# LahiruCooray/rl-aerial-manipulator

Hardware: NVIDIA B200
Metric: env_steps_per_sec (higher is better)
Workload: dtype f32

## Files before the change

### rl-aerial-manipulator_b200/csrc/qs_rollout_impl.cuh

```cuda
#include "../../include/quadsim.h"
#include "qs_internal.cuh"
#include "qs_tc.cuh"

#include <stdio.h>

#if !defined(QS_RO_NS) || !defined(QS_RO_EPI_SPLIT) || !defined(QS_RO_ENV_SPLIT) || !(defined(QS_RO_BUILD_FUSED) || defined(QS_RO_BUILD_POLICY))
#error "include qs_rollout_impl.cuh from qs_rollout.cu / qs_rollout_policy.cu"
#endif

namespace qs {
namespace QS_RO_NS {
using namespace tc;

constexpr int EPI_SPLIT = QS_RO_EPI_SPLIT, ENV_SPLIT = QS_RO_ENV_SPLIT;
constexpr int HEAD_SPLIT = EPI_SPLIT < 2 ? EPI_SPLIT : 2;
__host__ __device__ constexpr int chunk_owner(int ch) { return EPI_SPLIT == 3 ? (ch < 4 ? ch % 3 : (ch - 3) % 3) : ch % EPI_SPLIT; }
constexpr int EPI_WARPS = 8 * EPI_SPLIT, ENV_WARPS = 4 * ENV_SPLIT, MMA_WARPS = 2;
#ifndef QS_RO_ENV_FIRST
#define QS_RO_ENV_FIRST 0
#endif
#ifndef QS_RO_LDBUF
#define QS_RO_LDBUF 1
#endif
#ifndef QS_RO_LD_SPLIT
#define QS_RO_LD_SPLIT 0
#endif
#ifndef QS_RO_ST16
#ifdef QS_RO_BUILD_POLICY
#define QS_RO_ST16 1
#else
#define QS_RO_ST16 0
#endif
#endif
constexpr int W_EPI0 = QS_RO_ENV_FIRST ? ENV_WARPS : 0, W_ENV0 = QS_RO_ENV_FIRST ? 0 : EPI_WARPS, W_MMA0 = EPI_WARPS + ENV_WARPS;
constexpr int RO_WARPS = ((EPI_WARPS + ENV_WARPS + MMA_WARPS + 3) / 4) * 4;
constexpr int RO_THREADS = RO_WARPS * 32;
constexpr int REGS_LAUNCH = (65536 / RO_THREADS) / 8 * 8;
#ifdef QS_RO_BUILD_FUSED
constexpr bool REBALANCE = REGS_LAUNCH < 128;
#else
constexpr bool REBALANCE = false;
#endif
constexpr int REGS_MMA = 40;
constexpr int REGS_ENV = EPI_SPLIT == 1 ? 128 : 152;
constexpr int REGS_EPI = EPI_SPLIT == 1 ? 88 : 72;
static_assert(!REBALANCE || (EPI_WARPS * REGS_EPI + ENV_WARPS * REGS_ENV + 4 * REGS_MMA) * 32 <= RO_THREADS * REGS_LAUNCH, "register pool of the CTA");
static_assert(!REBALANCE || (EPI_WARPS % 4 == 0 && ENV_WARPS % 4 == 0), "setmaxnreg works on whole warpgroups");
constexpr int XBUFS = ENV_SPLIT == 2 ? 2 : 3;

constexpr uint32_t SLOT_COLS = 256, C_D1 = 0, C_D2 = 128, C_D3 = 192;

constexpr int IMG_WHI = 0, IMG_WLO = W_SET, IMG_CONST = 2 * W_SET;
constexpr int IMG_BYTES = IMG_CONST + ((C_TOTAL * 4 + 127) / 128) * 128;
constexpr int X_HALF = (K1 / 8) * ROWS * 16;
constexpr int X_BYTES = 2 * X_HALF;
constexpr int ONE_BYTES = 2 * ROWS * 16;
constexpr int X_LBO = ROWS * 16;
constexpr int SM_ONE = IMG_BYTES;
constexpr int SM_X = SM_ONE + ONE_BYTES;
constexpr int SM_OUT_MEAN = SM_X + XBUFS * X_BYTES;
constexpr int SM_OUT_VAL = SM_OUT_MEAN + 2 * HEAD_SPLIT * ROWS * 16;
constexpr int SM_TILE = SM_OUT_VAL + 2 * HEAD_SPLIT * ROWS * 4;
constexpr int SM_MOM = SM_TILE + ENV_WARPS * 32 * 21 * 4;
constexpr int SM_NORM = SM_MOM + ENV_WARPS * 40 * 8;
constexpr int SM_BARS = SM_NORM + 3 * 32 * 4;
enum : int { B_XFULL = 0 , B_XFREE = 3 , B_D1 = 6, B_D2 = 8, B_D3 = 10, B_H1 = 12, B_H2 = 20, B_D3FREE = 24, B_OUTF = 26, B_OUTE = 34, N_BARS = 42 };
constexpr int SM_MISC = SM_BARS + N_BARS * 8;
constexpr int SM_TOTAL = SM_MISC + 16;
static_assert(SM_TOTAL <= 232448, "shared memory budget of one CTA on B200");
static_assert(SM_X % 128 == 0 && SM_ONE % 128 == 0, "operand tiles are 128-byte aligned");

__device__ int g_ro_status;

#ifdef QS_RO_TRACE
constexpr int TRACE_LEN = 2048;
__device__ uint2 g_ro_trace[32][TRACE_LEN];
#define RO_TRACE_INIT() uint2* tr_buf = g_ro_trace[threadIdx.x >> 5]; int tr_n = 0; const bool tr_on = blockIdx.x == 0 && (threadIdx.x & 31) == 0
#define RO_TRACE(code) do { if (tr_on && tr_n < TRACE_LEN - 1) tr_buf[tr_n++] = make_uint2((uint32_t)(code), (uint32_t)clock64()); } while (0)
#define RO_TRACE_END() do { if (tr_on) tr_buf[TRACE_LEN - 1] = make_uint2((uint32_t)tr_n, 0u); } while (0)
#else
#define RO_TRACE_INIT() do { } while (0)
#define RO_TRACE(code) do { } while (0)
#define RO_TRACE_END() do { } while (0)
#endif

struct RoParams {
    const unsigned char* image;
    const float* params;
    const float* obs;
    const double* norm;
    float norm_eps, norm_clip;
    int sample_mode;
    const float* noise;
    uint64_t noise_seed;
    unsigned long long* noise_step;
    float lo[4], hi[4];
    float* obs_norm_out;
    float* actions;
    float* actions_clipped;
    float* values;
    float* logp;
    int64_t n;
    StepParams<float> sp;
    double* mom_out;
    double* mom_merge;
    unsigned int* ticket;
};

__device__ __forceinline__ void mbar_arrive(uint32_t bar) {
    asm volatile("mbarrier.arrive.shared::cta.b64 _, [%0];" ::"r"(bar) : "memory");
}
#ifndef QS_RO_WAIT_HINT_NS
#define QS_RO_WAIT_HINT_NS 20000
#endif
#ifndef QS_RO_BACKOFF_NS
#define QS_RO_BACKOFF_NS 0
#endif
__device__ __forceinline__ uint32_t mbar_try(uint32_t bar, uint32_t parity) {
    uint32_t ok;
#if QS_RO_WAIT_HINT_NS > 0
    asm volatile(
        "{\n\t"
        ".reg .pred p;\n\t"
        "mbarrier.try_wait.parity.shared::cta.b64 p, [%1], %2, %3;\n\t"
        "selp.u32 %0, 1, 0, p;\n\t"
        "}\n"
        : "=r"(ok)
        : "r"(bar), "r"(parity), "r"((uint32_t)QS_RO_WAIT_HINT_NS)
        : "memory");
#else
    asm volatile(
        "{\n\t"
        ".reg .pred p;\n\t"
        "mbarrier.try_wait.parity.shared::cta.b64 p, [%1], %2;\n\t"
        "selp.u32 %0, 1, 0, p;\n\t"
        "}\n"
        : "=r"(ok)
        : "r"(bar), "r"(parity)
        : "memory");
#endif
    return ok;
}
__device__ __forceinline__ uint32_t mbar_test(uint32_t bar, uint32_t parity) {
    uint32_t ok;
    asm volatile(
        "{\n\t"
        ".reg .pred p;\n\t"
        "mbarrier.test_wait.parity.shared::cta.b64 p, [%1], %2;\n\t"
        "selp.u32 %0, 1, 0, p;\n\t"
        "}\n"
        : "=r"(ok)
        : "r"(bar), "r"(parity)
        : "memory");
    return ok;
}
#ifndef QS_RO_TIGHT_WAIT
#define QS_RO_TIGHT_WAIT 1
#endif
__device__ __forceinline__ bool mbar_wait_slow(uint32_t bar, uint32_t parity, int code) {
#if QS_RO_TIGHT_WAIT
    uint32_t ok;
    asm volatile(
        "{\n\t"
        ".reg .pred p, q;\n\t"
        ".reg .u32 n;\n\t"
        "mov.u32 n, 0;\n\t"
        "QS_WAIT_LOOP:\n\t"
        "mbarrier.try_wait.parity.shared::cta.b64 p, [%1], %2, %3;\n\t"
        "@p bra QS_WAIT_DONE;\n\t"
        "add.u32 n, n, 1;\n\t"
        "setp.lt.u32 q, n, 4194304;\n\t"
        "@q bra QS_WAIT_LOOP;\n\t"
        "QS_WAIT_DONE:\n\t"
        "selp.u32 %0, 1, 0, p;\n\t"
        "}\n"
        : "=r"(ok)
        : "r"(bar), "r"(parity), "r"((uint32_t)(QS_RO_WAIT_HINT_NS > 0 ? QS_RO_WAIT_HINT_NS : 1000))
        : "memory");
    if (ok) return true;
#else
    for (uint32_t it = 0; it < (1u << 17); ++it) {
#if QS_RO_BACKOFF_NS > 0
        __nanosleep(QS_RO_BACKOFF_NS);
#endif
        if (mbar_try(bar, parity)) return true;
        if ((it & 0xFF) == 0xFF && *reinterpret_cast<volatile int*>(&g_ro_status) != 0) break;
    }
#endif
    atomicCAS(&g_ro_status, 0, code);
    return false;
}
__device__ __forceinline__ bool mbar_wait_bounded(uint32_t bar, uint32_t parity, int code) {
    if (mbar_try(bar, parity)) return true;
    return mbar_wait_slow(bar, parity, code);
}
#ifndef QS_RO_LAZY_WAIT_NS
#define QS_RO_LAZY_WAIT_NS 600
#endif
__device__ __forceinline__ bool mbar_wait_lazy(uint32_t bar, uint32_t parity, int code) {
#if QS_RO_LAZY_WAIT_NS > 0
    if (mbar_test(bar, parity)) return true;
    for (uint32_t it = 0; it < (1u << 22); ++it) {
        __nanosleep(QS_RO_LAZY_WAIT_NS);
        if (mbar_test(bar, parity)) return true;
    }
    atomicCAS(&g_ro_status, 0, code);
    return false;
#else
    return mbar_wait_bounded(bar, parity, code);
#endif
}
__device__ __forceinline__ void umma_ss(uint32_t tmem_d, uint64_t adesc, uint64_t bdesc, uint32_t idesc, uint32_t accumulate) {
    asm volatile(
        "{\n\t"
        ".reg .pred p;\n\t"
        "setp.ne.b32 p, %4, 0;\n\t"
        "tcgen05.mma.cta_group::1.kind::f16 [%0], %1, %2, %3, p;\n\t"
        "}\n" ::"r"(tmem_d), "l"(adesc), "l"(bdesc), "r"(idesc), "r"(accumulate)
        : "memory");
}
__device__ __forceinline__ void split_h2_rn(float a, float b, uint32_t& hi, uint32_t& lo) {
    asm("cvt.rn.f16x2.f32 %0, %1, %2;" : "=r"(hi) : "f"(b), "f"(a));
#ifdef QS_X_NOSPLIT
    lo = hi ^ 0x3C003C00u;
    return;
#endif
#ifdef QS_X_TRUNCSPLIT
    split_h2(a, b, hi, lo);
    return;
#endif
    float la, lb;
    asm("{\n\t"
        ".reg .f16 l, h, m;\n\t"
        "mov.b32 {l, h}, %2;\n\t"
        "mov.b16 m, 0xBC00;\n\t"
        "fma.rn.f32.f16 %0, l, m, %3;\n\t"
        "fma.rn.f32.f16 %1, h, m, %4;\n\t"
        "}\n"
        : "=f"(la), "=f"(lb)
        : "r"(hi), "f"(a), "f"(b));
    asm("cvt.rn.f16x2.f32 %0, %1, %2;" : "=r"(lo) : "f"(lb), "f"(la));
}
__device__ __forceinline__ void put32_rn(uint32_t taddr, const float* y) {
    uint32_t h[16], l[16];
#pragma unroll
    for (int j = 0; j < 16; ++j) split_h2_rn(y[2 * j], y[2 * j + 1], h[j], l[j]);
    tmem_st16(taddr, h);
    tmem_st16(taddr + 16, l);
}

struct Ctx {
    uint32_t sbase;
    uint32_t tmem;
    int cnt;
    __device__ __forceinline__ uint32_t bar(int idx) const { return sbase + SM_BARS + 8u * (uint32_t)idx; }
};

__device__ __forceinline__ void issue_l1(const Ctx& c, uint32_t d1, int xb, int net) {
    const uint32_t idesc = make_idesc(N1);
    const uint32_t xa = c.sbase + SM_X + xb * X_BYTES;
    const uint32_t wh = c.sbase + IMG_WHI + OFF_W1 + net * W1_BYTES, wl = c.sbase + IMG_WLO + OFF_W1 + net * W1_BYTES;
    constexpr uint32_t B_LBO = N1 * 16;
#pragma unroll
    for (int ks = 0; ks < K1 / 16; ++ks) {
        const uint64_t ah = make_desc(xa + ks * 2 * X_LBO, X_LBO, 128), al = make_desc(xa + X_HALF + ks * 2 * X_LBO, X_LBO, 128);
        const uint64_t bh = make_desc(wh + ks * 2 * B_LBO, B_LBO, 128), bl = make_desc(wl + ks * 2 * B_LBO, B_LBO, 128);
        umma_ss(d1, ah, bh, idesc, ks ? 1u : 0u);
        umma_ss(d1, ah, bl, idesc, 1);
        umma_ss(d1, al, bh, idesc, 1);
    }
}
__device__ __forceinline__ void issue_bias(const Ctx& c, uint32_t d, uint32_t wh, uint32_t wl, int bias_ks) {
    constexpr uint32_t B_LBO = N2 * 16;
    const uint32_t idesc = make_idesc(N2);
    const uint64_t one = make_desc(c.sbase + SM_ONE, X_LBO, 128);
    umma_ss(d, one, make_desc(wh + bias_ks * 2 * B_LBO, B_LBO, 128), idesc, 0);
    umma_ss(d, one, make_desc(wl + bias_ks * 2 * B_LBO, B_LBO, 128), idesc, 1);
}
__device__ __forceinline__ void issue_chunk(uint32_t d, uint32_t a_col, int ch, uint32_t wh, uint32_t wl) {
    constexpr uint32_t B_LBO = N2 * 16;
    const uint32_t idesc = make_idesc(N2);
#pragma unroll
    for (int j = 0; j < 2; ++j) {
        const int ks = 2 * ch + j;
        const uint32_t a_hi = a_col + 32u * ch + (QS_RO_LD_SPLIT ? 16u : 8u) * j;
        const uint64_t bh = make_desc(wh + ks * 2 * B_LBO, B_LBO, 128), bl = make_desc(wl + ks * 2 * B_LBO, B_LBO, 128);
        umma_ts(d, a_hi, bh, idesc, 1);
        umma_ts(d, a_hi, bl, idesc, 1);
        umma_ts(d, a_hi + (QS_RO_LD_SPLIT ? 8u : 16u), bh, idesc, 1);
    }
}

__device__ __forceinline__ void role_mma(const Ctx& c, int slot) {
    const uint32_t d1 = c.tmem + slot * SLOT_COLS + C_D1, d2 = c.tmem + slot * SLOT_COLS + C_D2, d3 = c.tmem + slot * SLOT_COLS + C_D3;
    const int role = 300 + slot * 50;
    uint32_t job = 0;
    bool l1_issued = false;
    RO_TRACE_INIT();
    for (int i = slot; i < c.cnt; i += 2) {
        const int xb = i % XBUFS;
#pragma unroll 1
        for (int net = 0; net < 2; ++net, ++job) {
            const uint32_t par = job & 1u;
            const uint32_t w2h = c.sbase + IMG_WHI + OFF_W2 + net * W2_BYTES, w2l = c.sbase + IMG_WLO + OFF_W2 + net * W2_BYTES;
            const uint32_t w3h = c.sbase + IMG_WHI + OFF_W3 + net * W3_BYTES, w3l = c.sbase + IMG_WLO + OFF_W3 + net * W3_BYTES;
            if (!l1_issued) {
                if (net == 0 && !mbar_wait_bounded(c.bar(B_XFULL + xb), (uint32_t)(i / XBUFS) & 1u, role + B_XFULL + 1)) return;
                tc_fence_after();
                if (elect_one()) {
                    issue_l1(c, d1, xb, net);
                    umma_commit(c.bar(B_D1 + slot));
                    if (net == 1) umma_commit(c.bar(B_XFREE + xb));
                }
                __syncwarp();
                RO_TRACE(0x200000u | job);
            }
            l1_issued = false;
            if (elect_one()) issue_bias(c, d2, w2h, w2l, N1 / 16);
            __syncwarp();
#pragma unroll 1
            for (int ch = 0; ch < 4; ++ch) {
                if (!mbar_wait_bounded(c.bar(B_H1 + slot * 4 + ch), par, role + B_H1 + 1)) return;
                RO_TRACE(0x210000u | (ch << 12) | job);
                tc_fence_after();
                if (elect_one()) {
                    issue_chunk(d2, d1, ch, w2h, w2l);
                    if (ch == 3) umma_commit(c.bar(B_D2 + slot));
                }
                __syncwarp();
            }
            RO_TRACE(0x220000u | job);
            int nxb = xb, nnet = 1, ni = i;
            bool have_next = true;
            if (net == 1) { ni = i + 2; nnet = 0; nxb = ni % XBUFS; have_next = ni < c.cnt; }
            bool l1_now = have_next && (net == 0 || mbar_test(c.bar(B_XFULL + nxb), (uint32_t)(ni / XBUFS) & 1u));
            l1_now = __shfl_sync(0xffffffffu, l1_now ? 1 : 0, 0) != 0;
            if (l1_now) {
                tc_fence_after();
                if (elect_one()) {
                    issue_l1(c, d1, nxb, nnet);
                    umma_commit(c.bar(B_D1 + slot));
                    if (nnet == 1) umma_commit(c.bar(B_XFREE + nxb));
                }
                __syncwarp();
                l1_issued = true;
                RO_TRACE(0x230000u | job);
            }
            if (!mbar_wait_bounded(c.bar(B_D3FREE + slot), par ^ 1u, role + B_D3FREE + 1)) return;
            RO_TRACE(0x240000u | job);
            tc_fence_after();
            if (elect_one()) issue_bias(c, d3, w3h, w3l, N2 / 16);
            __syncwarp();
#pragma unroll 1
            for (int ch = 0; ch < 2; ++ch) {
                if (!mbar_wait_bounded(c.bar(B_H2 + slot * 2 + ch), par, role + B_H2 + 1)) return;
                RO_TRACE(0x250000u | (ch << 12) | job);
                tc_fence_after();
                if (elect_one()) {
                    issue_chunk(d3, d2, ch, w3h, w3l);
                    if (ch == 1) umma_commit(c.bar(B_D3 + slot));
                }
                __syncwarp();
            }
            RO_TRACE(0x260000u | job);
        }
    }
    RO_TRACE_END();
}

__device__ __forceinline__ void tmem_st4(uint32_t taddr, const uint32_t* v) {
    asm volatile("tcgen05.st.sync.aligned.32x32b.x4.b32 [%0], {%1, %2, %3, %4};\n" ::"r"(taddr), "r"(v[0]), "r"(v[1]), "r"(v[2]), "r"(v[3]) : "memory");
}
__device__ __forceinline__ void tmem_ld16(uint32_t taddr, uint32_t* v) {
    asm volatile(
        "tcgen05.ld.sync.aligned.32x32b.x16.b32 {%0, %1, %2, %3, %4, %5, %6, %7, %8, %9, %10, %11, %12, %13, %14, %15}, [%16];\n"
        : "=r"(v[0]), "=r"(v[1]), "=r"(v[2]), "=r"(v[3]), "=r"(v[4]), "=r"(v[5]), "=r"(v[6]), "=r"(v[7]), "=r"(v[8]), "=r"(v[9]),
          "=r"(v[10]), "=r"(v[11]), "=r"(v[12]), "=r"(v[13]), "=r"(v[14]), "=r"(v[15])
        : "r"(taddr));
}
__device__ __forceinline__ void tmem_ld_wait16(uint32_t* v) {
    asm volatile("tcgen05.wait::ld.sync.aligned;"
                 : "+r"(v[0]), "+r"(v[1]), "+r"(v[2]), "+r"(v[3]), "+r"(v[4]), "+r"(v[5]), "+r"(v[6]), "+r"(v[7]), "+r"(v[8]), "+r"(v[9]),
                   "+r"(v[10]), "+r"(v[11]), "+r"(v[12]), "+r"(v[13]), "+r"(v[14]), "+r"(v[15])
                 :
                 : "memory");
}
__device__ __forceinline__ void tanh_split8(const uint32_t* v, uint32_t hi_col, uint32_t lo_col) {
    float y[8];
    tanh8_from_exponents(v, y);
    uint32_t h[4], l[4];
#pragma unroll
    for (int j = 0; j < 4; ++j) split_h2_rn(y[2 * j], y[2 * j + 1], h[j], l[j]);
    tmem_st4(hi_col, h);
    tmem_st4(lo_col, l);
}
__device__ __forceinline__ void chunk_tanh_split(uint32_t col) {
    uint32_t v[32];
#if QS_RO_LD_SPLIT
    tmem_ld16(col, v);
    tmem_ld_wait16(v);
    tmem_ld16(col + 16u, v + 16);
    tanh_split8(v, col, col + 8u);
    tanh_split8(v + 8, col + 4u, col + 12u);
    tmem_ld_wait16(v + 16);
    tanh_split8(v + 16, col + 16u, col + 24u);
    tanh_split8(v + 24, col + 20u, col + 28u);
#else
    tmem_ld32(col, v);
    tmem_ld_wait32(v);
#if QS_RO_ST16
    uint32_t h[16], l[16];
#pragma unroll
    for (int sb = 0; sb < 4; ++sb) {
        float y[8];
        tanh8_from_exponents(v + 8 * sb, y);
#pragma unroll
        for (int j = 0; j < 4; ++j) split_h2_rn(y[2 * j], y[2 * j + 1], h[4 * sb + j], l[4 * sb + j]);
    }
    asm volatile(
        "{\n\t"
        ".reg .b32 a2;\n\t"
        "add.u32 a2, %0, 16;\n\t"
        "tcgen05.st.sync.aligned.32x32b.x16.b32 [%0], {%1, %2, %3, %4, %5, %6, %7, %8, %9, %10, %11, %12, %13, %14, %15, %16};\n\t"
        "tcgen05.st.sync.aligned.32x32b.x16.b32 [a2], {%17, %18, %19, %20, %21, %22, %23, %24, %25, %26, %27, %28, %29, %30, %31, %32};\n\t"
        "}\n" ::"r"(col),
        "r"(h[0]), "r"(h[1]), "r"(h[2]), "r"(h[3]), "r"(h[4]), "r"(h[5]), "r"(h[6]), "r"(h[7]), "r"(h[8]), "r"(h[9]), "r"(h[10]), "r"(h[11]), "r"(h[12]),
        "r"(h[13]), "r"(h[14]), "r"(h[15]), "r"(l[0]), "r"(l[1]), "r"(l[2]), "r"(l[3]), "r"(l[4]), "r"(l[5]), "r"(l[6]), "r"(l[7]), "r"(l[8]), "r"(l[9]),
        "r"(l[10]), "r"(l[11]), "r"(l[12]), "r"(l[13]), "r"(l[14]), "r"(l[15])
        : "memory");
#else
#pragma unroll
    for (int sb = 0; sb < 4; ++sb) tanh_split8(v + 8 * sb, col + 4u * sb, col + 16u + 4u * sb);
#endif
#endif
}

#ifndef QS_RO_DEFER_HEAD
#define QS_RO_DEFER_HEAD 1
#endif
#ifndef QS_RO_HEAD_SCALAR_VF
#ifdef QS_RO_BUILD_POLICY
#define QS_RO_HEAD_SCALAR_VF 1
#else
#define QS_RO_HEAD_SCALAR_VF 0
#endif
#endif
__device__ __forceinline__ void role_epilogue(const Ctx& c, int slot, int half, int quad, int lane, const float* sC, float4* s_mean, float* s_val) {
    const uint32_t tm = c.tmem + slot * SLOT_COLS + ((uint32_t)(quad * 32) << 16);
    const int role = 100 + slot * 50;
    const int row = quad * 32 + lane;
    const uint32_t njobs = c.cnt > slot ? 2u * (uint32_t)((c.cnt - slot + 1) / 2) : 0u;
    float mean[NACT] = {0.f, 0.f, 0.f, 0.f};
    RO_TRACE_INIT();
#pragma unroll 1
    for (uint32_t job = 0; job < njobs + QS_RO_DEFER_HEAD; ++job) {
        const uint32_t par = job & 1u;
        const bool live = job < njobs;
#pragma unroll 1
        for (int stage = 0; stage < 3; ++stage) {
            if (stage == (QS_RO_DEFER_HEAD ? 1 : 2)) {
                if (QS_RO_DEFER_HEAD ? job == 0 : !live) continue;
                if (half >= HEAD_SPLIT) continue;
                const uint32_t hj = job - QS_RO_DEFER_HEAD, hpar = hj & 1u;
                const int net = (int)(hj & 1u);
                const uint32_t k = hj >> 1;
                if (!mbar_wait_bounded(c.bar(B_D3 + slot), hpar, role + B_D3 + 1)) return;
                RO_TRACE(0x130000u | hj);
                tc_fence_after();
                float o[NACT];
#pragma unroll
                for (int j = 0; j < NACT; ++j) o[j] = half == 0 ? sC[C_BH + net * NACT + j] : 0.f;
#pragma unroll 1
                for (int ch = half; ch < 2; ch += HEAD_SPLIT) {
                    uint32_t v[32];
                    tmem_ld32(tm + C_D3 + 32u * (uint32_t)ch, v);
                    tmem_ld_wait32(v);
                    if (ch + HEAD_SPLIT >= 2) {
                        tc_fence_before();
                        __syncwarp();
                        if (lane == 0) mbar_arrive(c.bar(B_D3FREE + slot));
                    }
                    const float4* wh = reinterpret_cast<const float4*>(sC + C_WH + net * N3 * NACT) + 32 * ch;
#pragma unroll
                    for (int sb = 0; sb < 4; ++sb) {
                        float y[8];
                        tanh8_from_exponents(v + 8 * sb, y);
#if QS_RO_HEAD_SCALAR_VF
                        if (net == 1) {
                            const float* w1 = reinterpret_cast<const float*>(wh + 8 * sb);
#pragma unroll
                            for (int q = 0; q < 8; ++q) o[0] = fmaf(y[q], w1[4 * q], o[0]);
                        } else
#endif
                        {
#pragma unroll
                            for (int q = 0; q < 8; ++q) {
                                const float4 w = wh[8 * sb + q];
                                o[0] = fmaf(y[q], w.x, o[0]); o[1] = fmaf(y[q], w.y, o[1]); o[2] = fmaf(y[q], w.z, o[2]); o[3] = fmaf(y[q], w.w, o[3]);
                            }
                        }
                    }
                }
                RO_TRACE(0x140000u | hj);
                if (net == 0) {
#pragma unroll
                    for (int j = 0; j < NACT; ++j) mean[j] = o[j];
                } else {
                    if (!mbar_wait_bounded(c.bar(B_OUTE + slot * 4 + quad), (k & 1u) ^ 1u, role + B_OUTE + 1)) return;
                    s_mean[(slot * HEAD_SPLIT + half) * ROWS + row] = make_float4(mean[0], mean[1], mean[2], mean[3]);
                    s_val[(slot * HEAD_SPLIT + half) * ROWS + row] = o[0];
                    __syncwarp();
                    if (lane == 0) mbar_arrive(c.bar(B_OUTF + slot * 4 + quad));
                }
            } else {
                if (!live) continue;
                const bool first = stage == 0;
                if (EPI_SPLIT == 3 && !first && half == 0) continue;
                if (!mbar_wait_bounded(c.bar((first ? B_D1 : B_D2) + slot), par, role + (first ? B_D1 : B_D2) + 1)) return;
                tc_fence_after();
#pragma unroll 1
                for (int ch = (first ? 0 : 4); ch < (first ? 4 : 6); ++ch) {
                    if (chunk_owner(ch) != half) continue;
                    RO_TRACE(0x100000u | (ch << 12) | job);
                    chunk_tanh_split(tm + 32u * (uint32_t)ch);
                    tmem_st_wait();
                    tc_fence_before();
                    __syncwarp();
                    if (lane == 0) mbar_arrive(c.bar(first ? B_H1 + slot * 4 + ch : B_H2 + slot * 2 + (ch - 4)));
                    RO_TRACE(0x110000u | (ch << 12) | job);
                }
            }
        }
    }
    RO_TRACE_END();
}

__device__ __forceinline__ float4 philox_normal4(uint64_t seed, uint64_t gid, unsigned long long step) {
    uint32_t w[4];
    philox4x32_10((uint32_t)gid, (uint32_t)(gid >> 32), (uint32_t)step, (uint32_t)(step >> 32), (uint32_t)seed ^ 0x85A308D3u,
                  (uint32_t)(seed >> 32) ^ 0x243F6A88u, w);
    float z[4];
#pragma unroll
    for (int j = 0; j < 2; ++j) {
        const float u1 = ((float)(w[2 * j] >> 9) + 0.5f) * 1.1920928955078125e-07f;
        const float th = (float)(w[2 * j + 1] >> 8) * 3.7450702829239286e-07f;
        const float r = sqrtf(-1.3862943611198906f * __log2f(u1));
        float s, co;
        __sincosf(th, &s, &co);
        z[2 * j] = r * co;
        z[2 * j + 1] = r * s;
    }
    return make_float4(z[0], z[1], z[2], z[3]);
}

template <int OBS>
__device__ __forceinline__ bool stage_x(const Ctx& c, const RoParams& p, int i, int quad, int lane, unsigned char* smem, const float* s_norm) {
    const int xb = i % XBUFS;
    if (!mbar_wait_bounded(c.bar(B_XFREE + xb), ((uint32_t)(i / XBUFS) & 1u) ^ 1u, 200 + B_XFREE + 1)) return false;
    const int row = quad * 32 + lane;
    const int64_t tile = (int64_t)blockIdx.x + (int64_t)i * gridDim.x;
    const int64_t e = tile * ROWS + row;
    float x[K1];
#pragma unroll
    for (int k = 0; k < K1; ++k) x[k] = 0.f;
    if (e < p.n) {
        const float* src = p.obs + e * OBS;
        if (OBS % 4 == 0) {
#pragma unroll
            for (int k = 0; k < OBS / 4; ++k) {
                const float4 q = __ldcs(reinterpret_cast<const float4*>(src) + k);
                x[4 * k] = q.x; x[4 * k + 1] = q.y; x[4 * k + 2] = q.z; x[4 * k + 3] = q.w;
            }
        } else {
#pragma unroll
            for (int k = 0; k < OBS; ++k) x[k] = __ldcs(src + k);
        }
        const int64_t e_pf = e + (int64_t)3 * gridDim.x * ROWS;
        if (e_pf < p.n) {
            const char* nr = reinterpret_cast<const char*>(p.obs + e_pf * OBS);
            asm volatile("prefetch.global.L2 [%0];" ::"l"(nr));
            asm volatile("prefetch.global.L2 [%0];" ::"l"(nr + OBS * 4 - 4));
// ... 154 lines not shown
            const int rows = rem < 32 ? (rem < 0 ? 0 : (int)rem) : 32;
            if (rows > 0) warp_store_rows<OBS>(sp.obs_out + e0 * OBS, tile_s, lane, rows);
            if (moments && lane < OBS && rows > 0) {
                const float L = tile_s[lane];
                double t1 = 0.0, t2 = 0.0;
#pragma unroll
                for (int r0 = 0; r0 < 32; r0 += 8) {
                    float a1 = 0.f, a2 = 0.f;
#pragma unroll
                    for (int r = r0; r < r0 + 8; ++r) {
                        const float v = r < rows ? tile_s[r * (OBS + 1) + lane] - L : 0.f;
                        a1 += v;
                        a2 = fmaf(v, v, a2);
                    }
                    t1 += (double)a1;
                    t2 += (double)a2;
                }
                const double dl = (double)L - G;
                m1 += t1 + (double)rows * dl;
                m2 += t2 + 2.0 * dl * t1 + (double)rows * dl * dl;
            }
            __syncwarp();
        }
    }
    if (moments && lane < OBS) { s_mom[lane] = m1; s_mom[OBS + lane] = m2; }
    RO_TRACE_END();
}

template <int VER, bool FUSED>
__global__ void __launch_bounds__(RO_THREADS, 1) rollout_kernel(const RoParams p) {
    constexpr int OBS = EnvTraits<VER>::OBS;
    extern __shared__ __align__(128) unsigned char smem[];
    const int tid = threadIdx.x, warp = tid >> 5, lane = tid & 31;
    float* sC = reinterpret_cast<float*>(smem + IMG_CONST);
    float4* s_mean = reinterpret_cast<float4*>(smem + SM_OUT_MEAN);
    float* s_val = reinterpret_cast<float*>(smem + SM_OUT_VAL);
    float* s_norm = reinterpret_cast<float*>(smem + SM_NORM);
    uint32_t* s_misc = reinterpret_cast<uint32_t*>(smem + SM_MISC);

    if (warp == 0) {
        asm volatile("tcgen05.alloc.cta_group::1.sync.aligned.shared::cta.b32 [%0], %1;" ::"r"(smem_u32(s_misc)), "r"(TMEM_COLS));
        asm volatile("tcgen05.relinquish_alloc_permit.cta_group::1.sync.aligned;" ::);
    }
    if (tid == 32) {
        const uint32_t b = smem_u32(smem + SM_BARS);
        for (int j = 0; j < N_BARS; ++j) {
            uint32_t count = 1u;
            if ((j >= B_XFULL && j < B_XFULL + 3) || (j >= B_H1 && j < B_D3FREE)) count = 4u;
            if (j >= B_D3FREE && j < B_D3FREE + 2) count = 4u * HEAD_SPLIT;
            if (j >= B_OUTF && j < B_OUTF + 8) count = HEAD_SPLIT;
            tc::mbar_init(b + 8u * j, count);
        }
        asm volatile("fence.mbarrier_init.release.cluster;" ::: "memory");
    }
    if (p.image) {
        const uint4* src = reinterpret_cast<const uint4*>(p.image);
        uint4* dst = reinterpret_cast<uint4*>(smem);
        for (int j = tid; j < IMG_BYTES / 16; j += RO_THREADS) dst[j] = __ldg(src + j);
    } else {
        const Blob B{OBS};
        for (int net = 0; net < 2; ++net) {
            const float sc = 2.8853900817779268f;
            stage_weights<true, RO_THREADS>(p.params + B.w1(net), p.params + B.b1(net), OBS, OBS, K1, N1, sc, smem + IMG_WHI + OFF_W1 + net * W1_BYTES,
                                            smem + IMG_WLO + OFF_W1 + net * W1_BYTES, tid);
            stage_weights<true, RO_THREADS>(p.params + B.w2(net), p.params + B.b2(net), N1, N1, N1 + KB, N2, sc, smem + IMG_WHI + OFF_W2 + net * W2_BYTES,
                                            smem + IMG_WLO + OFF_W2 + net * W2_BYTES, tid);
            stage_weights<true, RO_THREADS>(p.params + B.w3(net), p.params + B.b3(net), N2, N2, N2 + KB, N3, sc, smem + IMG_WHI + OFF_W3 + net * W3_BYTES,
                                            smem + IMG_WLO + OFF_W3 + net * W3_BYTES, tid);
            for (int j = tid; j < N3 * NACT; j += RO_THREADS) sC[C_WH + net * N3 * NACT + j] = __ldg(p.params + B.wh(net) + j);
            if (tid < NACT) sC[C_BH + net * NACT + tid] = __ldg(p.params + B.bh(net) + tid);
        }
        if (tid < NACT) sC[C_LS + tid] = __ldg(p.params + B.log_std() + tid);
    }
    for (int j = tid; j < ONE_BYTES / 16; j += RO_THREADS)
        reinterpret_cast<uint4*>(smem + SM_ONE)[j] = j < ROWS ? make_uint4(0x00003C00u, 0u, 0u, 0u) : make_uint4(0u, 0u, 0u, 0u);
    if (tid < 32) {
        double m = 0.0, is = 1.0;
        if (p.norm && tid < OBS) {
            m = p.norm[1 + tid];
            is = 1.0 / sqrt(p.norm[1 + OBS + tid] + (double)p.norm_eps);
        }
        s_norm[tid] = (float)m;
        s_norm[32 + tid] = (float)(m - (double)(float)m);
        s_norm[64 + tid] = (float)is;
    }
    unsigned long long noise_step = 0;
    if (p.sample_mode == 2 && p.noise_step) noise_step = *reinterpret_cast<const volatile unsigned long long*>(p.noise_step);
    fence_async_smem();
    tc_fence_before();
    __syncthreads();
    tc_fence_after();

    Ctx c;
    c.sbase = smem_u32(smem);
    c.tmem = s_misc[0];
    const int64_t n_tiles = (p.n + ROWS - 1) / ROWS;
    c.cnt = (int)((n_tiles - blockIdx.x + gridDim.x - 1) / gridDim.x);

    if (warp >= W_EPI0 && warp < W_EPI0 + EPI_WARPS) {
        if (REBALANCE && REGS_EPI > REGS_LAUNCH) asm volatile("setmaxnreg.inc.sync.aligned.u32 %0;" ::"n"(REGS_EPI));
        if (REBALANCE && REGS_EPI < REGS_LAUNCH) asm volatile("setmaxnreg.dec.sync.aligned.u32 %0;" ::"n"(REGS_EPI));
        role_epilogue(c, (warp - W_EPI0) / (4 * EPI_SPLIT), ((warp - W_EPI0) >> 2) % EPI_SPLIT, warp & 3, lane, sC, s_mean, s_val);
        if (REBALANCE && REGS_EPI > REGS_LAUNCH) asm volatile("setmaxnreg.dec.sync.aligned.u32 %0;" ::"n"(REGS_LAUNCH));
        if (REBALANCE && REGS_EPI < REGS_LAUNCH) asm volatile("setmaxnreg.inc.sync.aligned.u32 %0;" ::"n"(REGS_LAUNCH));
    } else if (warp >= W_ENV0 && warp < W_ENV0 + ENV_WARPS) {
        if (REBALANCE) asm volatile("setmaxnreg.inc.sync.aligned.u32 %0;" ::"n"(REGS_ENV));
        role_env<VER, FUSED>(c, p, ENV_SPLIT == 2 ? (warp - W_ENV0) >> 2 : 0, warp & 3, lane, smem, sC, s_mean, s_val, noise_step);
        if (REBALANCE) asm volatile("setmaxnreg.dec.sync.aligned.u32 %0;" ::"n"(REGS_LAUNCH));
    } else {
        if (REBALANCE) asm volatile("setmaxnreg.dec.sync.aligned.u32 %0;" ::"n"(REGS_MMA));
        if (warp < W_MMA0 + MMA_WARPS) role_mma(c, warp - W_MMA0);
        if (REBALANCE) asm volatile("setmaxnreg.inc.sync.aligned.u32 %0;" ::"n"(REGS_LAUNCH));
    }
    tc_fence_before();
    __syncthreads();
    if (warp == 0) {
        tc_fence_after();
        asm volatile("tcgen05.dealloc.cta_group::1.sync.aligned.b32 %0, %1;" ::"r"(c.tmem), "r"(TMEM_COLS));
    }
    if (!FUSED) {
        if (p.sample_mode == 2 && p.noise_step) {
            __threadfence();
            __syncthreads();
            if (tid == 0) s_misc[1] = atomicAdd(p.ticket, 1u) == gridDim.x - 1 ? 1u : 0u;
            __syncthreads();
            if (s_misc[1] != 0u && tid == 0) {
                *p.ticket = 0u;
                *p.noise_step = noise_step + 1ull;
            }
        }
        return;
    }

    const StepParams<float>& sp = p.sp;
    const bool moments = sp.mom_partial != nullptr;
    if (moments && tid < 2 * OBS) {
        const double* sm = reinterpret_cast<const double*>(smem + SM_MOM);
        double a = 0.0;
#pragma unroll
        for (int w = 0; w < ENV_WARPS; ++w) a += sm[w * 40 + tid];
        sp.mom_partial[(int64_t)blockIdx.x * 2 * OBS + tid] = a;
    }
    __threadfence();
    __syncthreads();
    if (tid == 0) s_misc[1] = atomicAdd(p.ticket, 1u) == gridDim.x - 1 ? 1u : 0u;
    __syncthreads();
    if (s_misc[1] == 0u) return;
    __threadfence();
    if (tid == 0) {
        *p.ticket = 0u;
        if (p.sample_mode == 2 && p.noise_step) *p.noise_step = noise_step + 1ull;
    }
    if (!moments) return;
    double* red = reinterpret_cast<double*>(smem);
    constexpr int W2 = 2 * OBS, SL = RO_THREADS / W2;
    const int col = tid % W2, slice = tid / W2;
    double shift = 0.0;
    if (tid < OBS) shift = p.mom_out[0] > 0.0 ? p.mom_out[1 + tid] : (sp.mom_stats ? sp.mom_stats[1 + tid] : 0.0);
    if (slice < SL) {
        double acc = 0.0;
        for (int b = slice; b < (int)gridDim.x; b += SL) acc += __ldcg(sp.mom_partial + (int64_t)b * W2 + col);
        red[slice * W2 + col] = acc;
    }
    __syncthreads();
    const double cnt = (double)p.n;
    double mean_b = 0.0, m2_b = 0.0, count = 0.0, mean_r = 0.0, var_r = 0.0;
    if (tid < OBS) {
        double s1 = 0.0, s2 = 0.0;
        for (int k = 0; k < SL; ++k) { s1 += red[k * W2 + tid]; s2 += red[k * W2 + OBS + tid]; }
        mean_b = shift + s1 / cnt;
        m2_b = s2 - s1 * s1 / cnt;
        if (p.mom_merge) {
// ... 50 lines not shown

}

#ifdef QS_RO_BUILD_POLICY
int launch_policy_pipeline(const float* params, int obs_dim, const float* obs, const float* noise, int64_t n, const double* norm_stats,
                           float norm_eps, float norm_clip, float* obs_norm_out, float* actions, float* actions_clipped,
                           const float* clip_lo, const float* clip_hi, float* values, float* logp, cudaStream_t stream,
                           const char** err_out, uint64_t philox_seed, uint64_t* philox_counter, int64_t env_id_offset) {
    static thread_local char msg[256];
    QS_RO_NS::RoParams p;
    memset(&p, 0, sizeof(p));
    p.params = params; p.obs = obs; p.norm = norm_stats; p.norm_eps = norm_eps; p.norm_clip = norm_clip;
    p.sample_mode = noise ? 1 : 0; p.noise = noise;
    if (philox_counter) {
        p.sample_mode = 2; p.noise = nullptr; p.noise_seed = philox_seed;
        p.noise_step = reinterpret_cast<unsigned long long*>(philox_counter);
        p.ticket = reinterpret_cast<unsigned int*>(philox_counter + 1);
        p.sp.env_id_offset = env_id_offset;
    }
    for (int i = 0; i < 4; ++i) { p.lo[i] = clip_lo ? clip_lo[i] : -3.4e38f; p.hi[i] = clip_hi ? clip_hi[i] : 3.4e38f; }
    p.obs_norm_out = obs_norm_out; p.actions = actions; p.actions_clipped = actions_clipped; p.values = values; p.logp = logp; p.n = n;
    int dev = 0, sms = 0;
    cudaGetDevice(&dev);
    cudaDeviceGetAttribute(&sms, cudaDevAttrMultiProcessorCount, dev);
    const cudaError_t err = obs_dim == 20 ? QS_RO_NS::launch<ENV_V2, false>(p, sms, stream) : QS_RO_NS::launch<ENV_V1, false>(p, sms, stream);
    if (err != cudaSuccess) {
        snprintf(msg, sizeof(msg), "rollout_kernel<policy only>: %s", cudaGetErrorString(err));
        *err_out = msg;
        return QS_ECUDA;
    }
    return QS_OK;
}


int policy_pipeline_status() {
    int v = 0;
    if (cudaMemcpyFromSymbol(&v, QS_RO_NS::g_ro_status, sizeof(int)) != cudaSuccess) return -1;
    if (v != 0) {
        const int zero = 0;
        cudaMemcpyToSymbol(QS_RO_NS::g_ro_status, &zero, sizeof(int));
    }
    return v;
}
#endif
}
#ifdef QS_RO_TRACE
#ifdef QS_RO_BUILD_POLICY
extern "C" int qs_trace_dump_policy(void* out, int bytes) {
#else
extern "C" int qs_trace_dump_fused(void* out, int bytes) {
#endif
    cudaDeviceSynchronize();
    return (int)cudaMemcpyFromSymbol(out, qs::QS_RO_NS::g_ro_trace, bytes < (int)sizeof(qs::QS_RO_NS::g_ro_trace) ? bytes : sizeof(qs::QS_RO_NS::g_ro_trace));
}
#endif
namespace qs {

#ifdef QS_RO_BUILD_FUSED
int policy_pipeline_status();
#endif
}

#ifdef QS_RO_BUILD_FUSED
using namespace qs;

extern "C" {

int64_t qs_policy_image_bytes(void) { return QS_RO_NS::IMG_BYTES; }

int qs_policy_prepare(const float* params, int obs_dim, void* image_out, void* stream) {
    if (!params || !image_out || (obs_dim != 20 && obs_dim != 17)) { set_error(nullptr, "qs_policy_prepare: bad argument (obs_dim 17 or 20)"); return QS_EINVAL; }
    if (reinterpret_cast<uintptr_t>(image_out) & 15) { set_error(nullptr, "qs_policy_prepare: image_out must be 16-byte aligned"); return QS_EINVAL; }
    cudaMemsetAsync(image_out, 0, QS_RO_NS::IMG_BYTES, (cudaStream_t)stream);
    if (obs_dim == 20) QS_RO_NS::policy_prepare_kernel<20><<<8, 256, 0, (cudaStream_t)stream>>>(params, (unsigned char*)image_out);
    else QS_RO_NS::policy_prepare_kernel<17><<<8, 256, 0, (cudaStream_t)stream>>>(params, (unsigned char*)image_out);
    const cudaError_t err = cudaGetLastError();
    if (err != cudaSuccess) { set_error(nullptr, "qs_policy_prepare: %s", cudaGetErrorString(err)); return QS_ECUDA; }
    return QS_OK;
}

int qs_rollout_step(qs_handle* h, const qs_rollout_args* a, void* stream) {
    if (!h || !a) { set_error(h, "qs_rollout_step: null argument"); return QS_EINVAL; }
    if (h->cfg.precision != QS_F32 || h->cfg.integrator != QS_RK4) { set_error(h, "qs_rollout_step: float32 / RK4 handles only"); return QS_EINVAL; }
    if (!h->initialized) { set_error(h, "qs_rollout_step: call qs_reset first"); return QS_EINVAL; }
    if (h->dyn_on) { set_error(h, "qs_rollout_step: the fused rollout kernel has no dynamics randomisation; use qs_policy_forward + qs_step, or disarm qs_dynamics_randomization"); return QS_EINVAL; }
    if (!a->policy_image || !a->obs || !a->obs_next || !a->actions_out || !a->values_out || !a->logp_out || !a->reward_out || !a->flags_out) {
        set_error(h, "qs_rollout_step: policy_image, obs, obs_next, actions_out, values_out, logp_out, reward_out and flags_out are required");
        return QS_EINVAL;
    }
    if (a->sample_mode < QS_SAMPLE_MEAN || a->sample_mode > QS_SAMPLE_PHILOX || (a->sample_mode == QS_SAMPLE_NOISE && !a->noise) ||
        (a->sample_mode == QS_SAMPLE_PHILOX && !a->noise_step)) {
        set_error(h, "qs_rollout_step: sample_mode needs its noise buffer (QS_SAMPLE_NOISE) or device step counter (QS_SAMPLE_PHILOX)");
        return QS_EINVAL;
    }
    const uintptr_t al = reinterpret_cast<uintptr_t>(a->policy_image) | reinterpret_cast<uintptr_t>(a->actions_out) | reinterpret_cast<uintptr_t>(a->noise) |
                         reinterpret_cast<uintptr_t>(a->actions_clipped_out) | reinterpret_cast<uintptr_t>(a->obs) | reinterpret_cast<uintptr_t>(a->obs_next) |
                         reinterpret_cast<uintptr_t>(a->obs_norm_out);
    if (al & 15) { set_error(h, "qs_rollout_step: image, obs, noise and action buffers must be 16-byte aligned"); return QS_EINVAL; }
    cudaError_t err = cudaSetDevice(h->cfg.device);
    if (err != cudaSuccess) { set_error(h, "qs_rollout_step: cudaSetDevice: %s", cudaGetErrorString(err)); return QS_ECUDA; }
    if (!h->ro_ticket) {
        err = cudaMalloc(&h->ro_ticket, sizeof(unsigned int));
        if (err == cudaSuccess) err = cudaMemset(h->ro_ticket, 0, sizeof(unsigned int));
        if (err != cudaSuccess) { set_error(h, "qs_rollout_step: ticket allocation: %s", cudaGetErrorString(err)); return QS_ECUDA; }
    }
    QS_RO_NS::RoParams p;
// ... 33 lines not shown
```

Baseline: 3.157 billion.

## Replace epilogue-to-MMA mbarrier handoffs with hardware named barriers

```diff
diff --git a/rl-aerial-manipulator_b200/csrc/qs_ro_schedule.h b/rl-aerial-manipulator_b200/csrc/qs_ro_schedule.h
--- /dev/null
+++ b/rl-aerial-manipulator_b200/csrc/qs_ro_schedule.h
@@ -0,0 +1,24 @@
+#pragma once
+
+#if defined(__CUDACC__)
+#define QS_RO_HD __host__ __device__
+#else
+#define QS_RO_HD
+#endif
+
+namespace qs {
+namespace ro_sched {
+
+QS_RO_HD constexpr int chunk_owner(int ch, int epi_split) { return epi_split == 3 ? (ch < 4 ? ch % 3 : (ch - 3) % 3) : ch % epi_split; }
+QS_RO_HD constexpr int head_split(int epi_split) { return epi_split < 2 ? epi_split : 2; }
+QS_RO_HD constexpr int slot_jobs(int cnt, int slot) { return cnt > slot ? 2 * ((cnt - slot + 1) / 2) : 0; }
+
+QS_RO_HD constexpr int nb_chunk(int slot, int ch) { return 1 + 6 * slot + ch; }
+QS_RO_HD constexpr int nb_d3free(int slot) { return 13 + slot; }
+constexpr int NB_LAST = 14;
+static_assert(NB_LAST < 16, "sixteen hardware barriers per CTA");
+QS_RO_HD constexpr int nb_chunk_threads() { return 32 + 4 * 32; }
+QS_RO_HD constexpr int nb_d3free_threads(int epi_split) { return 32 + 4 * head_split(epi_split) * 32; }
+
+}
+}
diff --git a/rl-aerial-manipulator_b200/csrc/qs_rollout_impl.cuh b/rl-aerial-manipulator_b200/csrc/qs_rollout_impl.cuh
--- a/rl-aerial-manipulator_b200/csrc/qs_rollout_impl.cuh
+++ b/rl-aerial-manipulator_b200/csrc/qs_rollout_impl.cuh
@@ -1,6 +1,7 @@
 #include "../../include/quadsim.h"
 #include "qs_internal.cuh"
 #include "qs_tc.cuh"
+#include "qs_ro_schedule.h"
 
 #include <stdio.h>
 
@@ -13,8 +14,8 @@
 using namespace tc;
 
 constexpr int EPI_SPLIT = QS_RO_EPI_SPLIT, ENV_SPLIT = QS_RO_ENV_SPLIT;
-constexpr int HEAD_SPLIT = EPI_SPLIT < 2 ? EPI_SPLIT : 2;
-__host__ __device__ constexpr int chunk_owner(int ch) { return EPI_SPLIT == 3 ? (ch < 4 ? ch % 3 : (ch - 3) % 3) : ch % EPI_SPLIT; }
+constexpr int HEAD_SPLIT = ro_sched::head_split(EPI_SPLIT);
+__host__ __device__ constexpr int chunk_owner(int ch) { return ro_sched::chunk_owner(ch, EPI_SPLIT); }
 constexpr int EPI_WARPS = 8 * EPI_SPLIT, ENV_WARPS = 4 * ENV_SPLIT, MMA_WARPS = 2;
 #ifndef QS_RO_ENV_FIRST
 #define QS_RO_ENV_FIRST 0
@@ -82,6 +83,20 @@
 #define RO_TRACE_INIT() do { } while (0)
 #define RO_TRACE(code) do { } while (0)
 #define RO_TRACE_END() do { } while (0)
+#endif
+
+#ifdef QS_RO_COUNT
+enum : int { CNT_WAITS = 0, CNT_POLLS, CNT_LAZY_WAITS, CNT_LAZY_POLLS, CNT_NBAR_SYNCS, NCNT };
+constexpr int CNT_ROLES = 3, CNT_MAX_CTAS = 1024;
+__device__ unsigned int g_ro_count[CNT_MAX_CTAS][CNT_ROLES][4][NCNT];
+__shared__ unsigned int s_ro_count[CNT_ROLES][4][NCNT];
+__device__ __forceinline__ int count_role() {
+    const int w = (int)(threadIdx.x >> 5);
+    return (w >= W_EPI0 && w < W_EPI0 + EPI_WARPS) ? 0 : (w >= W_ENV0 && w < W_ENV0 + ENV_WARPS) ? 1 : 2;
+}
+#define RO_COUNT(k, v) do { if ((threadIdx.x & 31) == 0) atomicAdd(&s_ro_count[count_role()][(threadIdx.x >> 5) & 3][k], (unsigned)(v)); } while (0)
+#else
+#define RO_COUNT(k, v) do { } while (0)
 #endif
 
 struct RoParams {
@@ -160,6 +175,29 @@
 __device__ __forceinline__ bool mbar_wait_slow(uint32_t bar, uint32_t parity, int code) {
 #if QS_RO_TIGHT_WAIT
     uint32_t ok;
+#ifdef QS_RO_COUNT
+    uint32_t polls;
+    asm volatile(
+        "{\n\t"
+        ".reg .pred p, q;\n\t"
+        ".reg .u32 n;\n\t"
+        "mov.u32 n, 0;\n\t"
+        "QS_WAIT_LOOP:\n\t"
+        "mbarrier.try_wait.parity.shared::cta.b64 p, [%2], %3, %4;\n\t"
+        "@p bra QS_WAIT_DONE;\n\t"
+        "add.u32 n, n, 1;\n\t"
+        "setp.lt.u32 q, n, 4194304;\n\t"
+        "@q bra QS_WAIT_LOOP;\n\t"
+        "QS_WAIT_DONE:\n\t"
+        "selp.u32 %0, 1, 0, p;\n\t"
+        "mov.u32 %1, n;\n\t"
+        "}\n"
+        : "=r"(ok), "=r"(polls)
+        : "r"(bar), "r"(parity), "r"((uint32_t)(QS_RO_WAIT_HINT_NS > 0 ? QS_RO_WAIT_HINT_NS : 1000))
+        : "memory");
+    RO_COUNT(CNT_POLLS, polls + 1u);
+    if (ok) RO_COUNT(CNT_WAITS, 1);
+#else
     asm volatile(
         "{\n\t"
         ".reg .pred p, q;\n\t"
@@ -177,6 +215,7 @@
         : "=r"(ok)
         : "r"(bar), "r"(parity), "r"((uint32_t)(QS_RO_WAIT_HINT_NS > 0 ? QS_RO_WAIT_HINT_NS : 1000))
         : "memory");
+#endif
     if (ok) return true;
 #else
     for (uint32_t it = 0; it < (1u << 17); ++it) {
@@ -191,7 +230,12 @@
     return false;
 }
 __device__ __forceinline__ bool mbar_wait_bounded(uint32_t bar, uint32_t parity, int code) {
-    if (mbar_try(bar, parity)) return true;
+    if (mbar_try(bar, parity)) {
+        RO_COUNT(CNT_POLLS, 1);
+        RO_COUNT(CNT_WAITS, 1);
+        return true;
+    }
+    RO_COUNT(CNT_POLLS, 1);
     return mbar_wait_slow(bar, parity, code);
 }
 #ifndef QS_RO_LAZY_WAIT_NS
@@ -199,16 +243,31 @@
 #endif
 __device__ __forceinline__ bool mbar_wait_lazy(uint32_t bar, uint32_t parity, int code) {
 #if QS_RO_LAZY_WAIT_NS > 0
-    if (mbar_test(bar, parity)) return true;
+    RO_COUNT(CNT_LAZY_POLLS, 1);
+    if (mbar_test(bar, parity)) { RO_COUNT(CNT_LAZY_WAITS, 1); return true; }
     for (uint32_t it = 0; it < (1u << 22); ++it) {
         __nanosleep(QS_RO_LAZY_WAIT_NS);
-        if (mbar_test(bar, parity)) return true;
+        RO_COUNT(CNT_LAZY_POLLS, 1);
+        if (mbar_test(bar, parity)) { RO_COUNT(CNT_LAZY_WAITS, 1); return true; }
     }
     atomicCAS(&g_ro_status, 0, code);
     return false;
 #else
     return mbar_wait_bounded(bar, parity, code);
 #endif
+}
+#ifndef QS_RO_NAMED_BAR
+#define QS_RO_NAMED_BAR 1
+#endif
+__device__ __forceinline__ void nbar_arrive(int id, int threads) {
+    asm volatile("bar.arrive %0, %1;" ::"r"(id), "r"(threads) : "memory");
+}
+__device__ __forceinline__ bool nbar_wait(uint32_t abort_flag, int id, int threads) {
+    asm volatile("bar.sync %0, %1;" ::"r"(id), "r"(threads) : "memory");
+    RO_COUNT(CNT_NBAR_SYNCS, 1);
+    uint32_t a;
+    asm volatile("ld.volatile.shared.u32 %0, [%1];" : "=r"(a) : "r"(abort_flag) : "memory");
+    return a == 0u;
 }
 __device__ __forceinline__ void umma_ss(uint32_t tmem_d, uint64_t adesc, uint64_t bdesc, uint32_t idesc, uint32_t accumulate) {
     asm volatile(
@@ -254,7 +313,49 @@
     uint32_t tmem;
     int cnt;
     __device__ __forceinline__ uint32_t bar(int idx) const { return sbase + SM_BARS + 8u * (uint32_t)idx; }
+    __device__ __forceinline__ uint32_t abort_flag() const { return sbase + SM_MISC + 8u; }
 };
+
+__device__ __forceinline__ bool wait_chunk_stored(const Ctx& c, int slot, int ch, uint32_t par, int role) {
+#if QS_RO_NAMED_BAR
+    return nbar_wait(c.abort_flag(), ro_sched::nb_chunk(slot, ch), ro_sched::nb_chunk_threads());
+#else
+    return ch < 4 ? mbar_wait_bounded(c.bar(B_H1 + slot * 4 + ch), par, role + B_H1 + 1)
+                  : mbar_wait_bounded(c.bar(B_H2 + slot * 2 + (ch - 4)), par, role + B_H2 + 1);
+#endif
+}
+__device__ __forceinline__ void signal_chunk_stored(const Ctx& c, int slot, int ch, int lane) {
+#if QS_RO_NAMED_BAR
+    nbar_arrive(ro_sched::nb_chunk(slot, ch), ro_sched::nb_chunk_threads());
+#else
+    __syncwarp();
+    if (lane == 0) mbar_arrive(c.bar(ch < 4 ? B_H1 + slot * 4 + ch : B_H2 + slot * 2 + (ch - 4)));
+#endif
+}
+__device__ __forceinline__ bool wait_d3_free(const Ctx& c, int slot, uint32_t job, int role) {
+#if QS_RO_NAMED_BAR
+    return job == 0 || nbar_wait(c.abort_flag(), ro_sched::nb_d3free(slot), ro_sched::nb_d3free_threads(EPI_SPLIT));
+#else
+    return mbar_wait_bounded(c.bar(B_D3FREE + slot), (job & 1u) ^ 1u, role + B_D3FREE + 1);
+#endif
+}
+__device__ __forceinline__ void signal_d3_free(const Ctx& c, int slot, int lane) {
+#if QS_RO_NAMED_BAR
+    nbar_arrive(ro_sched::nb_d3free(slot), ro_sched::nb_d3free_threads(EPI_SPLIT));
+#else
+    __syncwarp();
+    if (lane == 0) mbar_arrive(c.bar(B_D3FREE + slot));
+#endif
+}
+__device__ __forceinline__ void epi_abandon(const Ctx& c, int slot, int half) {
+#if QS_RO_NAMED_BAR
+    asm volatile("st.volatile.shared.u32 [%0], 1;" ::"r"(c.abort_flag()) : "memory");
+    __syncwarp();
+    for (int ch = 0; ch < 6; ++ch)
+        if (chunk_owner(ch) == half) nbar_arrive(ro_sched::nb_chunk(slot, ch), ro_sched::nb_chunk_threads());
+    if (half < HEAD_SPLIT) nbar_arrive(ro_sched::nb_d3free(slot), ro_sched::nb_d3free_threads(EPI_SPLIT));
+#endif
+}
 
 __device__ __forceinline__ void issue_l1(const Ctx& c, uint32_t d1, int xb, int net) {
     const uint32_t idesc = make_idesc(N1);
@@ -320,7 +421,7 @@
             __syncwarp();
 #pragma unroll 1
             for (int ch = 0; ch < 4; ++ch) {
-                if (!mbar_wait_bounded(c.bar(B_H1 + slot * 4 + ch), par, role + B_H1 + 1)) return;
+                if (!wait_chunk_stored(c, slot, ch, par, role)) return;
                 RO_TRACE(0x210000u | (ch << 12) | job);
                 tc_fence_after();
                 if (elect_one()) {
@@ -346,14 +447,14 @@
                 l1_issued = true;
                 RO_TRACE(0x230000u | job);
             }
-            if (!mbar_wait_bounded(c.bar(B_D3FREE + slot), par ^ 1u, role + B_D3FREE + 1)) return;
+            if (!wait_d3_free(c, slot, job, role)) return;
             RO_TRACE(0x240000u | job);
             tc_fence_after();
             if (elect_one()) issue_bias(c, d3, w3h, w3l, N2 / 16);
             __syncwarp();
 #pragma unroll 1
             for (int ch = 0; ch < 2; ++ch) {
-                if (!mbar_wait_bounded(c.bar(B_H2 + slot * 2 + ch), par, role + B_H2 + 1)) return;
+                if (!wait_chunk_stored(c, slot, 4 + ch, par, role)) return;
                 RO_TRACE(0x250000u | (ch << 12) | job);
                 tc_fence_after();
                 if (elect_one()) {
@@ -365,6 +466,9 @@
             RO_TRACE(0x260000u | job);
         }
     }
+#if QS_RO_NAMED_BAR
+    if (!wait_d3_free(c, slot, job, role)) return;
+#endif
     RO_TRACE_END();
 }
 
@@ -464,7 +568,7 @@
                 const uint32_t hj = job - QS_RO_DEFER_HEAD, hpar = hj & 1u;
                 const int net = (int)(hj & 1u);
                 const uint32_t k = hj >> 1;
-                if (!mbar_wait_bounded(c.bar(B_D3 + slot), hpar, role + B_D3 + 1)) return;
+                if (!mbar_wait_bounded(c.bar(B_D3 + slot), hpar, role + B_D3 + 1)) { epi_abandon(c, slot, half); return; }
                 RO_TRACE(0x130000u | hj);
                 tc_fence_after();
                 float o[NACT];
@@ -477,8 +581,7 @@
                     tmem_ld_wait32(v);
                     if (ch + HEAD_SPLIT >= 2) {
                         tc_fence_before();
-                        __syncwarp();
-                        if (lane == 0) mbar_arrive(c.bar(B_D3FREE + slot));
+                        signal_d3_free(c, slot, lane);
                     }
                     const float4* wh = reinterpret_cast<const float4*>(sC + C_WH + net * N3 * NACT) + 32 * ch;
 #pragma unroll
@@ -506,7 +609,7 @@
 #pragma unroll
                     for (int j = 0; j < NACT; ++j) mean[j] = o[j];
                 } else {
-                    if (!mbar_wait_bounded(c.bar(B_OUTE + slot * 4 + quad), (k & 1u) ^ 1u, role + B_OUTE + 1)) return;
+                    if (!mbar_wait_bounded(c.bar(B_OUTE + slot * 4 + quad), (k & 1u) ^ 1u, role + B_OUTE + 1)) { epi_abandon(c, slot, half); return; }
                     s_mean[(slot * HEAD_SPLIT + half) * ROWS + row] = make_float4(mean[0], mean[1], mean[2], mean[3]);
                     s_val[(slot * HEAD_SPLIT + half) * ROWS + row] = o[0];
                     __syncwarp();
@@ -516,7 +619,7 @@
                 if (!live) continue;
                 const bool first = stage == 0;
                 if (EPI_SPLIT == 3 && !first && half == 0) continue;
-                if (!mbar_wait_bounded(c.bar((first ? B_D1 : B_D2) + slot), par, role + (first ? B_D1 : B_D2) + 1)) return;
+                if (!mbar_wait_bounded(c.bar((first ? B_D1 : B_D2) + slot), par, role + (first ? B_D1 : B_D2) + 1)) { epi_abandon(c, slot, half); return; }
                 tc_fence_after();
 #pragma unroll 1
                 for (int ch = (first ? 0 : 4); ch < (first ? 4 : 6); ++ch) {
@@ -525,8 +628,7 @@
                     chunk_tanh_split(tm + 32u * (uint32_t)ch);
                     tmem_st_wait();
                     tc_fence_before();
-                    __syncwarp();
-                    if (lane == 0) mbar_arrive(c.bar(first ? B_H1 + slot * 4 + ch : B_H2 + slot * 2 + (ch - 4)));
+                    signal_chunk_stored(c, slot, ch, lane);
                     RO_TRACE(0x110000u | (ch << 12) | job);
                 }
             }
@@ -787,7 +889,11 @@
             tc::mbar_init(b + 8u * j, count);
         }
         asm volatile("fence.mbarrier_init.release.cluster;" ::: "memory");
-    }
+        s_misc[2] = 0u;
+    }
+#ifdef QS_RO_COUNT
+    if (tid < CNT_ROLES * 4 * NCNT) (&s_ro_count[0][0][0])[tid] = 0u;
+#endif
     if (p.image) {
         const uint4* src = reinterpret_cast<const uint4*>(p.image);
         uint4* dst = reinterpret_cast<uint4*>(smem);
@@ -853,6 +959,9 @@
         tc_fence_after();
         asm volatile("tcgen05.dealloc.cta_group::1.sync.aligned.b32 %0, %1;" ::"r"(c.tmem), "r"(TMEM_COLS));
     }
+#ifdef QS_RO_COUNT
+    if (tid < CNT_ROLES * 4 * NCNT && blockIdx.x < CNT_MAX_CTAS) (&g_ro_count[blockIdx.x][0][0][0])[tid] = (&s_ro_count[0][0][0])[tid];
+#endif
     if (!FUSED) {
         if (p.sample_mode == 2 && p.noise_step) {
             __threadfence();
@@ -1009,6 +1118,16 @@
 #endif
     cudaDeviceSynchronize();
     return (int)cudaMemcpyFromSymbol(out, qs::QS_RO_NS::g_ro_trace, bytes < (int)sizeof(qs::QS_RO_NS::g_ro_trace) ? bytes : sizeof(qs::QS_RO_NS::g_ro_trace));
+}
+#endif
+#ifdef QS_RO_COUNT
+#ifdef QS_RO_BUILD_POLICY
+extern "C" int qs_count_dump_policy(void* out, int bytes) {
+#else
+extern "C" int qs_count_dump_fused(void* out, int bytes) {
+#endif
+    cudaDeviceSynchronize();
+    return (int)cudaMemcpyFromSymbol(out, qs::QS_RO_NS::g_ro_count, bytes < (int)sizeof(qs::QS_RO_NS::g_ro_count) ? bytes : sizeof(qs::QS_RO_NS::g_ro_count));
 }
 #endif
 namespace qs {
```

After: 3.188 billion (median of 6 runs). Within noise of the previous version (+1.0%).
